# bderembl/msom

Measured on NVIDIA B200. Metric: cell-layer updates/s, higher is better.
Workload: dtype f64

## Files before the change

### include/msqg.h

```cpp
#ifndef MSQG_H
#define MSQG_H

#ifdef __cplusplus
extern "C" {
#endif

#define MSQG_MAXL 32

enum {
  MSQG_OK = 0,
  MSQG_ERR_ARG = -1,
  MSQG_ERR_CUDA = -2,
  MSQG_ERR_FILE = -3,
  MSQG_ERR_CONFIG = -4,
  MSQG_ERR_NOCONV = -5
};

typedef struct msqg_params {
  int N, nl, ediag, varRo, nptr, flsrv;
  double L0, Rom, Ekb, Eks, tau0, Re, Re4, sbc, beta, afilt, Lfmax;
  double DT, tend, dtout, dtflt, CFL;
  double Fr[MSQG_MAXL], dh[MSQG_MAXL], upg[MSQG_MAXL], vpg[MSQG_MAXL];
  double iRe, iRe4;
  int stochastic;
// ... 86 lines not shown
int msqg_filter_de_pm(msqg_model *m, double dtflt, double ediag, int pm_field);
int msqg_energy_tend(msqg_model *m, double dt, double ediag);
int msqg_reset_energy(msqg_model *m);
int msqg_tendency_bfn(msqg_model *m, double direction);
int msqg_bfn_direction(msqg_model *m, double direction);
double msqg_get_ts_previous(msqg_model *m);
void msqg_set_ts_previous(msqg_model *m, double v);
void msqg_seed_noise(msqg_model *m, unsigned seed);
int msqg_set_noise_mode(msqg_model *m, int mode);
long msqg_launch_count(msqg_model *m);
const char *msqg_last_error(void);

int msqg_set_keep_dq(msqg_model *m, int keep);
int msqg_set_dissipation(msqg_model *m, double iRe, double iRe4, double Eks, double Ekb);
void msqg_derive_params(msqg_params *p);

int msqg_test_relax(msqg_model *m, int level, double *a, const double *b, int nsweeps);
int msqg_test_relax_scalar(msqg_model *m, int level, double lambda, double *a, const double *b, int nsweeps);
int msqg_test_residual(msqg_model *m, const double *a, const double *b, double *res, double *maxres);
int msqg_test_residual_levels(msqg_model *m, int mode, const double *a, const double *b, double *out, double *maxres,
                              int *bottom);
int msqg_test_restrict(msqg_model *m, int level, const double *fine, double *coarse);
int msqg_test_prolong(msqg_model *m, int level, const double *coarse, double *fine);
int msqg_test_div(int device, const double *x, const double *d, double *q_fast, double *q_ieee, int n);
int msqg_profile_enable(msqg_model *m, int on);
int msqg_profile_read(msqg_model *m, double *ms, long *count, long *aux_sum);
int msqg_test_relax_profile(msqg_model *m, int level, int nsweeps, long long *out, int max_workers);
int msqg_time_vcycle(msqg_model *m, int nrelax, int reps, double *ms_out);

typedef struct msqg_ensemble msqg_ensemble;
int msqg_ensemble_create(const msqg_params *p, int device, int nmembers, const unsigned *seeds ,
                         int noise_mode, int smoother, msqg_ensemble **out);
void msqg_ensemble_destroy(msqg_ensemble *e);
int msqg_ensemble_size(msqg_ensemble *e);
msqg_model *msqg_ensemble_member(msqg_ensemble *e, int k);
int msqg_ensemble_set_const(msqg_ensemble *e);
int msqg_ensemble_step(msqg_ensemble *e, int nsteps, double *dt_last );
double msqg_ensemble_time(msqg_ensemble *e, int k);

typedef struct msqg_group msqg_group;
int msqg_nccl_unique_id(void *out128);
int msqg_group_create_local(const msqg_params *p, int device, int px, int py, int agg_n, msqg_group **out);
int msqg_group_create_nccl(const msqg_params *p, int device, int px, int py, int agg_n, int rank, int nranks,
                           const void *uid128, msqg_group **out);
int msqg_group_create_local_sm(const msqg_params *p, int device, int px, int py, int agg_n, int smoother, msqg_group **out);
int msqg_group_create_nccl_sm(const msqg_params *p, int device, int px, int py, int agg_n, int smoother, int rank, int nranks,
// ... 67 lines not shown
```

### msom_b200/capi.py

```python
import ctypes as C
import os

import numpy as np

_HERE = os.path.dirname(os.path.abspath(__file__))
LIB_CUDA = os.path.join(_HERE, "lib", "libmsqg_cuda.so")
MAXL = 32

(PSI, Q, PSIPG, FR, QFORC, TOPO, RD, SSTOCH, ZETA, DQ, STR, NSTOCH, IBU, CL2M, CM2L, PM, QM, TMP, ZETAP,
 QPRED, SIGFILT, DE_BF, DE_VD, DE_J1, DE_J2, DE_J3, DE_FT, PO_MFT, PTR, PTR_RELAX, DPTR, QOF, SIGLEV) = range(33)

OK, ERR_ARG, ERR_CUDA, ERR_FILE, ERR_CONFIG, ERR_NOCONV = 0, -1, -2, -3, -4, -5


class Params(C.Structure):
    _fields_ = (
        [(k, C.c_int) for k in ("N", "nl", "ediag", "varRo", "nptr", "flsrv")]
        + [(k, C.c_double) for k in ("L0", "Rom", "Ekb", "Eks", "tau0", "Re", "Re4", "sbc", "beta",
                                     "afilt", "Lfmax", "DT", "tend", "dtout", "dtflt", "CFL")]
        + [(k, C.c_double * MAXL) for k in ("Fr", "dh", "upg", "vpg")]
        + [("iRe", C.c_double), ("iRe4", C.c_double), ("stochastic", C.c_int),
           ("tr_stoch", C.c_double), ("itr_stoch", C.c_double), ("amp_stoch", C.c_double),
           ("mode_pv_invert", C.c_int)]
        + [(k, C.c_double * MAXL) for k in ("ptr_r", "Pe", "ptr_ir", "iPe")]
# ... 80 lines not shown
    L.msqg_invertq.argtypes = [vp, C.c_int]
    L.msqg_comp_q.argtypes = [vp]
    L.msqg_last_mgstats.argtypes = [vp, C.c_int, C.POINTER(MgStats)]
    L.msqg_total_cycles.argtypes = [vp]
    L.msqg_total_cycles.restype = C.c_long
    L.msqg_update.argtypes = [vp, C.c_int, C.c_double, pd]
    L.msqg_advance.argtypes = [vp, C.c_int, C.c_int, C.c_double]
    L.msqg_step.argtypes = [vp, C.c_double, C.c_double, pd, pd]
    L.msqg_ke1.argtypes = [vp, pd]
    L.msqg_tendency_bfn.argtypes = [vp, C.c_double]
    L.msqg_get_ts_previous.argtypes = [vp]
    L.msqg_get_ts_previous.restype = C.c_double
    L.msqg_set_ts_previous.argtypes = [vp, C.c_double]
    L.msqg_seed_noise.argtypes = [vp, C.c_uint]
    L.msqg_set_noise_mode.argtypes = [vp, C.c_int]
    L.msqg_launch_count.argtypes = [vp]
    L.msqg_launch_count.restype = C.c_long
    L.msqg_test_relax.argtypes = [vp, C.c_int, dp, dp, C.c_int]
    L.msqg_test_relax_scalar.argtypes = [vp, C.c_int, C.c_double, dp, dp, C.c_int]
    L.msqg_test_residual.argtypes = [vp, dp, dp, dp, pd]
    L.msqg_test_residual_levels.argtypes = [vp, C.c_int, dp, dp, dp, pd, C.POINTER(C.c_int)]
    L.msqg_test_restrict.argtypes = [vp, C.c_int, dp, dp]
    L.msqg_test_prolong.argtypes = [vp, C.c_int, dp, dp]
    L.msqg_test_div.argtypes = [C.c_int, dp, dp, dp, dp, C.c_int]
    L.msqg_time_vcycle.argtypes = [vp, C.c_int, C.c_int, pd]
    L.msqg_profile_enable.argtypes = [vp, C.c_int]
    L.msqg_profile_read.argtypes = [vp, pd, C.POINTER(C.c_long), C.POINTER(C.c_long)]
    L.msqg_reset_field.argtypes = [vp, C.c_int]
    _lib = L
    return L


def check(rc):
    if rc != 0:
        raise MsqgError(rc, lib().msqg_last_error().decode(errors="replace"))


def make_params(**kw):
    p = Params()
    lib().msqg_default_params(C.byref(p))
    for k, v in kw.items():
        if k in ("Fr", "dh", "upg", "vpg", "ptr_r", "Pe"):
            arr = getattr(p, k)
            for i, x in enumerate(v):
                arr[i] = float(x)
        else:
# ... 32 lines not shown
            if self.owned:
                self.L.msqg_destroy(self.h)
            self.h = None

    def __del__(self):
        try:
            self.close()
        except Exception:
            pass

    def nfields(self, fid):
        return self.L.msqg_nfields(self.h, fid)

    def set(self, fid, arr):
        arr = np.ascontiguousarray(arr, dtype=np.float64)
        assert arr.shape == (self.nfields(fid), self.N, self.N), (arr.shape, self.nfields(fid))
        check(self.L.msqg_set_field(self.h, fid, arr))

    def get(self, fid):
        out = np.zeros((self.nfields(fid), self.N, self.N))
        check(self.L.msqg_get_field(self.h, fid, out))
        return out

    def set_async(self, fid, pinned):
        check(self.L.msqg_set_field_async(self.h, fid, pinned))

    def commit(self):
        check(self.L.msqg_set_field_commit(self.h))

    def get_async(self, fid, pinned):
        check(self.L.msqg_get_field_async(self.h, fid, pinned))

    def io_wait(self):
        check(self.L.msqg_io_wait(self.h))

    def set_smoother(self, name):
        check(self.L.msqg_set_smoother(self.h, {"lex": 0, "rb": 1}[name]))

    def set_energy_conserv(self, on):
        check(self.L.msqg_set_energy_conserv(self.h, int(bool(on))))

    def set_const(self):
        check(self.L.msqg_set_const(self.h))

    def invertq(self, q_id=Q):
        check(self.L.msqg_invertq(self.h, q_id))
# ... 67 lines not shown
```

### msom_b200/csrc/model.cu

```cuda
#include "../../include/msqg.h"
#include "layout.cuh"
#include "mg_kernels.cuh"
#include "rb_kernels.cuh"
#include "rhs_kernels.cuh"

#include <cmath>
#include <cstdio>
#include <cstdlib>
#include <cstring>
#include <dlfcn.h>
#include <vector>
#include <utility>
#include <map>
#include <tuple>
#include <thread>
#include <mutex>
#include <condition_variable>
#include <string>
#include <atomic>

static thread_local char g_err[512] = "";
static std::mutex g_kernel_init_mu;
extern "C" const char *msqg_last_error(void) { return g_err; }
#define FAIL(code, ...)                        \
// ... 1147 lines not shown
static inline cudaError_t zero_words(cudaStream_t st, double *p, int n) {
  k_zero_words<<<1, 64, 0, st>>>(p, n);
  return cudaGetLastError();
}

static int check_relax_err(msqg_model *m) {
  CK(to_host(m->stream, m->h_err, m->d_err, 1));
  CK(cudaStreamSynchronize(m->stream));
  if (*m->h_err) {
    CK(cudaMemsetAsync(m->d_err, 0, sizeof(int), m->stream));
    k_fill_u64<<<m->num_sms * 4, 256, 0, m->stream>>>(m->mailbox, m->mailbox_words, MAIL_EMPTY);
    FAIL(MSQG_ERR_CUDA, "relax wavefront timed out waiting on a neighbour strip");
  }
  return MSQG_OK;
}

struct MgProblem {
  int nf;
  int mode;
  double *a;
  const double *b;
};

static int residual_pyr_bottom(const msqg_model *m) {
  const int D = m->depth;
  if (m->g[D].bc != 0 || m->periodic || D < 2) return D;
  return D - PYR_MAXLEV > 1 ? D - PYR_MAXLEV : 1;
}

static int mg_residual_enqueue(msqg_model *m, const MgProblem &P) {
  const int D = m->depth;
  const Geom &g = m->g[D];
  CK(zero_words(m->stream, m->d_scal, 1));
  const int bottom = residual_pyr_bottom(m);
  if (bottom < D) {
    PyrLevels L;
    L.nlev = D - bottom;
    for (int k = 0; k < PYR_MAXLEV; k++) {
      const int l = k < L.nlev ? D - 1 - k : D;
      L.p[k] = m->res.lev[l]; L.pitch[k] = m->g[l].pitch; L.plane[k] = m->g[l].plane; L.n[k] = m->g[l].nx;
    }
    const dim3 b(32, 8), grid((g.nx + PYR_TILE - 1) / PYR_TILE, (g.ny + PYR_TILE - 1) / PYR_TILE);
    const LayerMetrics M = metrics_of(m);
    StretchConsts S;
    for (int l = 0; l < MSQG_NLMAX; l++) S.s[l] = l < m->nl ? m->s_lev[(size_t)D * m->nl + l] : 0.;
    { ProfScope ps(m, PROF_RESIDUAL, 0);
    if (P.mode >= 0) {
      k_residual_pyr<1, true><<<grid, b, 0, m->stream>>>(P.a, P.b, m->res.lev[D], m->ibu.lev[D] + (size_t)P.mode * g.plane, S, g, M, L, m->d_scal);
    } else if (m->s_uniform) {
      NL_SWITCH(m->nl, k_residual_pyr<NL, false><<<grid, b, 0, m->stream>>>(P.a, P.b, m->res.lev[D], nullptr, S, g, M, L, m->d_scal));
    } else {
      NL_SWITCH(m->nl, k_residual_pyr<NL, true><<<grid, b, 0, m->stream>>>(P.a, P.b, m->res.lev[D], m->str.lev[D], S, g, M, L, m->d_scal));
    }
    }
    m->launches++;
    CK(cudaGetLastError());
    CK(to_host(m->stream, m->h_scal, m->d_scal, 1));
    return MSQG_OK;
  }
  dim3 b(64, 4);
  { ProfScope ps(m, PROF_RESIDUAL, 0);
  if (P.mode < 0) {
    LayerMetrics M = metrics_of(m);
    NL_SWITCH(m->nl, k_residual<NL><<<grid2(g.nx, g.ny, b), b, 0, m->stream>>>(P.a, P.b, m->res.lev[D], m->str.lev[D], g, M, m->d_scal));
  } else {
    k_residual_scalar<<<grid2(g.nx, g.ny, b), b, 0, m->stream>>>(P.a, P.b, m->res.lev[D], m->ibu.lev[D] + (size_t)P.mode * g.plane, g, m->d_scal);
  }
  }
// ... 196 lines not shown
      ModeMat<NL> M;
      for (int k = 0; k < NL * NL; k++) M.a[k] = m->h_cm2l[k];
      k_project<NL><<<grid2(g.nx, g.ny, b), b, 0, m->stream>>>(m->pm.lev[D], m->psi.lev[D], g, M, matf_m2l, 1);
    });
    m->launches++;
    CK(cudaGetLastError());
  }
  return MSQG_OK;
}
extern "C" int msqg_invertq(msqg_model *m, int q_id) {
  CK(cudaSetDevice(m->device));
  List *L = list_by_id(m, q_id);
  if (!L || L->nf != m->nl) FAIL(MSQG_ERR_ARG, "bad q list");
  if (m->group) return pg_invertq(m->group, m, q_id);
  return invertq_list(m, *L);
}

extern "C" int msqg_comp_q(msqg_model *m) {
  CK(cudaSetDevice(m->device));
  if (m->group) { int rc = pg_halo(m->group, MSQG_PSI); if (rc) return rc; }
  const Geom &g = m->g[m->depth];
  dim3 b(64, 4);
  LayerMetrics M = metrics_of(m);
  NL_SWITCH(m->nl, k_comp_q<NL><<<grid2(g.nx, g.ny, b), b, 0, m->stream>>>(m->psi.lev[m->depth], m->str.lev[m->depth], m->q.lev[m->depth], g, M));
  m->launches++;
  CK(cudaGetLastError());
  return MSQG_OK;
}

typedef void (*dgeev_fn)(const char *, const char *, const int *, double *, const int *, double *, double *, double *,
                         const int *, double *, const int *, double *, const int *, int *, size_t, size_t);
static dgeev_fn find_dgeev() {
  static dgeev_fn fn = nullptr;
  static bool tried = false;
  if (tried) return fn;
  tried = true;
  const char *cands[] = {getenv("MSQG_LAPACK"), "liblapack.so.3", "liblapack.so", "libopenblas.so.0", "libopenblas.so"};
  for (const char *c : cands) {
    if (!c) continue;
    void *h = dlopen(c, RTLD_NOW | RTLD_GLOBAL);
    if (!h) continue;
    fn = (dgeev_fn)dlsym(h, "dgeev_");
    if (!fn) fn = (dgeev_fn)dlsym(h, "scipy_dgeev_");
    if (fn) break;
  }
  return fn;
}
// ... 269 lines not shown
  return MSQG_OK;
}

extern "C" int msqg_set_const(msqg_model *m) {
  if (m->group) return pg_set_const(m->group);
  int rc = set_const_local(m);
  if (rc) return rc;
  return set_const_finish(m);
}

static double timestep_chain(msqg_model *m, double umax, double dtmax, double Delta) {
  const double CFL = m->p.CFL;
  dtmax /= CFL;
  if (umax != 0.) {
    const double dt = Delta / umax;
    if (dt < dtmax) dtmax = dt;
  }
  dtmax *= CFL;
  if (dtmax > m->ts_previous) dtmax = (m->ts_previous + 0.1 * dtmax) / 1.1;
  m->ts_previous = dtmax;
  return dtmax;
}

static int rhs_prepare(msqg_model *m) {
  const int D = m->depth;
  const Geom &g = m->g[D];
  dim3 b(64, 4);
  CK(zero_words(m->stream, m->d_scal + 1, m->nl));
  ProfScope ps(m, PROF_LAP, 0);
  launch_lap(m->stream, m->nl, m->psi.lev[D], m->zeta.lev[D], g, m->d_scal + 1, m->sbcc);
  m->launches++;
  if (m->iRe != 0. || m->iRe4 != 0.) {
    launch_lap(m->stream, m->nl, m->zeta.lev[D], m->tmp.lev[D], g, nullptr, m->sbcc);
    m->launches++;
  }
  CK(cudaGetLastError());
  CK(to_host(m->stream, m->h_scal + 1, m->d_scal + 1, m->nl));
  return MSQG_OK;
}
static double dt_chain(msqg_model *m, double dtmax) {
  const double Delta = m->g[m->depth].Delta;
  for (int l = 0; l < m->nl; l++) {
    dtmax = timestep_chain(m, m->h_scal[1 + l], dtmax, Delta);
    dtmax = timestep_chain(m, m->umax_pg[l], dtmax, Delta);
  }
  return dtmax;
}

static int rhs_launch(msqg_model *m, List &q_ev, const double *q_in, double *q_out, double *dq, double dt, float dts) {
  const int D = m->depth;
  const Geom &g = m->g[D];
  const int nl = m->nl;
  RhsArgs A;
  memset(&A, 0, sizeof(A));
  A.psi = m->psi.lev[D]; A.zeta = m->zeta.lev[D]; A.tmp = m->tmp.lev[D]; A.pp = m->psipg.lev[D];
  A.zp = m->zetap.lev[D]; A.s = m->str.lev[D]; A.qforc = m->has_qforc ? m->qforc.lev[D] : nullptr;
  A.topo = m->topo.lev[D]; A.ro = m->ro.lev[D];
  A.q_in = q_in; A.q_ev = q_ev.lev[D]; A.q_out = q_out; A.dq = dq;
  A.noise = m->p.stochastic ? m->nstoch.lev[D] : nullptr;
  A.wind = m->d_wind; A.g = g;
  for (int l = 0; l < nl; l++) { A.idh0[l] = m->idh0[l]; A.idh1[l] = m->idh1[l]; }
  A.beta = m->p.beta; A.iRe = m->iRe; A.iRe4 = m->iRe4;
  A.ceks = m->Eks / (m->p.Rom * 2 * m->dhf[0]);
  A.cekb = m->Ekb / (m->p.Rom * 2 * m->dhf[nl - 1]);
  A.dhb = m->dhf[nl - 1];
  A.dt = dt; A.itr = m->p.itr_stoch; A.dts = dts;
  A.has_pg = m->has_pg; A.has_zp = m->has_zp; A.use_tmp = (m->iRe != 0. || m->iRe4 != 0.);
  A.flag_topo = m->flag_topo; A.stochastic = m->p.stochastic;
  A.econs = (m->econs && !m->p.stochastic) ? 1 : 0;
  if (A.econs) {
    if (g.bc) FAIL(MSQG_ERR_ARG, "the ENERGY_CONSERV variant is not available on decomposed grids");
    dim3 bg(32, 8);
    k_ghosts<<<grid2(g.nx + 2, g.ny + 2, bg, nl), bg, 0, m->stream>>>(q_ev.lev[D], nl, g, -1.);
    m->launches++;
  }
  ProfScope ps(m, PROF_RHS, 0);
  static int rhs_variant = -1;
  if (rhs_variant < 0) { const char *e = getenv("MSQG_RHS"); rhs_variant = (e && !strcmp(e, "gather")) ? 0 : 1; }
  if (rhs_variant == 1 && !A.has_pg && !A.has_zp && !A.flag_topo && !A.stochastic && !A.econs) {
    dim3 bt(RT_X, RT_Y);
    NL_SWITCH(nl, k_rhs_t<NL><<<grid2(g.nx, g.ny, bt), bt, 0, m->stream>>>(A));
  } else {
    dim3 b(32, 4);
    NL_SWITCH(nl, k_rhs<NL><<<grid2(g.nx, g.ny, b), b, 0, m->stream>>>(A));
  }
  m->launches++;
  CK(cudaGetLastError());
  return MSQG_OK;
}

static int ptr_launch(msqg_model *m, List &tr, const double *tr_in, double *tr_out, double *dptr, double dt) {
  if (m->p.nptr <= 0) return MSQG_OK;
  if (m->g[m->depth].bc) FAIL(MSQG_ERR_ARG, "passive tracers are not supported on decomposed grids");
  const int D = m->depth;
  const Geom &g = m->g[D];
  PtrArgs A;
  memset(&A, 0, sizeof(A));
  A.psi = m->psi.lev[D]; A.ptr = tr.lev[D]; A.relax = m->ptr_relax.lev[D];
  A.ptr_in = tr_in; A.ptr_out = tr_out; A.dptr = dptr; A.g = g; A.dt = dt; A.nptr = m->p.nptr;
  for (int nt = 0; nt < m->p.nptr; nt++) { A.iPe[nt] = m->p.iPe[nt]; A.ptr_ir[nt] = m->p.ptr_ir[nt]; }
  dim3 b(64, 4);
  k_ptr_rhs<<<grid2(g.nx, g.ny, b, tr.nf), b, 0, m->stream>>>(A);
  m->launches++;
  CK(cudaGetLastError());
// ... 293 lines not shown
  launch_lap(m->stream, nl, m->psi.lev[D], m->zeta.lev[D], g, nullptr, m->sbcc);
  m->launches++;
  if (m->iRe != 0. || m->iRe4 != 0.) {
    launch_lap(m->stream, nl, m->zeta.lev[D], m->tmp.lev[D], g, nullptr, m->sbcc);
    m->launches++;
  }
  EnergyArgs A;
  memset(&A, 0, sizeof(A));
  A.psi = m->psi.lev[D]; A.zeta = m->zeta.lev[D]; A.tmp = m->tmp.lev[D]; A.pp = m->psipg.lev[D];
  A.zp = m->zetap.lev[D]; A.s = m->str.lev[D];
  A.de_bf = m->de_bf.lev[D]; A.de_vd = m->de_vd.lev[D]; A.de_j1 = m->de_j1.lev[D]; A.de_j2 = m->de_j2.lev[D];
  A.de_j3 = m->de_j3.lev[D]; A.po_mft = m->po_mft.lev[D];
  A.g = g;
  for (int l = 0; l < nl; l++) { A.idh0[l] = m->idh0[l]; A.idh1[l] = m->idh1[l]; }
  A.beta = m->p.beta; A.iRe = m->iRe; A.iRe4 = m->iRe4;
  A.ceks = m->Eks / (m->p.Rom * 2 * m->dhf[0]);
  A.cekb = m->Ekb / (m->p.Rom * 2 * m->dhf[nl - 1]);
  A.dt = dt; A.ediag = ediag;
  A.has_pg = m->has_pg; A.has_zp = m->has_zp; A.nme_ft = m->nme_ft;
  if (m->econs) {
    if (!m->tmp2.nf && (rc = alloc_list(m, m->tmp2, nl, -1., D, D))) return rc;
    dim3 bq(64, 4);
    LayerMetrics M = metrics_of(m);
    NL_SWITCH(nl, k_comp_q<NL><<<grid2(g.nx, g.ny, bq), bq, 0, m->stream>>>(m->psi.lev[D], m->str.lev[D], m->tmp2.lev[D], g, M));
    m->launches++;
    A.qt = m->tmp2.lev[D];
  }
  dim3 b(32, 4);
  NL_SWITCH(nl, k_energy<NL><<<grid2(g.nx, g.ny, b), b, 0, m->stream>>>(A));
  m->launches++;
  CK(cudaGetLastError());
  m->nme_ft += 1;
  return MSQG_OK;
}

extern "C" int msqg_ke1(msqg_model *m, double *ke) {
  CK(cudaSetDevice(m->device));
  const Geom &g = m->g[m->depth];
  dim3 b(16, 16);
  dim3 gr = grid2(g.nx, g.ny, b);
  k_ke_partial<<<gr, b, 0, m->stream>>>(m->psi.lev[m->depth], g, m->d_kepart);
  m->launches++;
  CK(cudaGetLastError());
  std::vector<double> part((size_t)gr.x * gr.y);
  CK(cudaMemcpyAsync(part.data(), m->d_kepart, part.size() * sizeof(double), cudaMemcpyDeviceToHost, m->stream));
  CK(cudaStreamSynchronize(m->stream));
  double s = 0.;
// ... 16 lines not shown
  CK(cudaStreamSynchronize(m->stream));
  (void)dt_chain(m, m->p.DT);
  return MSQG_OK;
}

static int upload_level(msqg_model *m, double *dst, const double *host, int nf, int lev, double sg) {
  const Geom &g = m->g[lev];
  size_t cnt = (size_t)nf * g.nx * g.ny;
  if (cnt > m->stage_doubles) FAIL(MSQG_ERR_ARG, "staging buffer too small");
  CK(cudaMemcpyAsync(m->d_stage, host, cnt * sizeof(double), cudaMemcpyHostToDevice, m->stream));
  dim3 b(32, 8);
  k_pack<<<grid2(g.nx + 2, g.ny + 2, b, nf), b, 0, m->stream>>>(dst, m->d_stage, nf, g, sg);
  CK(cudaGetLastError());
  CK(cudaStreamSynchronize(m->stream));
  return MSQG_OK;
}
static int download_level(msqg_model *m, double *host, const double *src, int nf, int lev) {
  const Geom &g = m->g[lev];
  size_t cnt = (size_t)nf * g.nx * g.ny;
  dim3 b(32, 8);
  k_unpack<<<grid2(g.nx, g.ny, b, nf), b, 0, m->stream>>>(m->d_stage, src, nf, g);
  CK(cudaGetLastError());
  CK(cudaMemcpyAsync(host, m->d_stage, cnt * sizeof(double), cudaMemcpyDeviceToHost, m->stream));
  CK(cudaStreamSynchronize(m->stream));
  return MSQG_OK;
}

extern "C" int msqg_test_relax(msqg_model *m, int level, double *a, const double *b, int nsweeps) {
  CK(cudaSetDevice(m->device));
  if (level < 1 || level > m->depth) FAIL(MSQG_ERR_ARG, "bad level");
  if (!m->const_set || !m->s_uniform) FAIL(MSQG_ERR_ARG, "needs set_const and uniform stretching");
  int rc;
  if ((rc = upload_level(m, m->da.lev[level], a, m->nl, level, -1.))) return rc;
  if ((rc = upload_level(m, m->res.lev[level], b, m->nl, level, -1.))) return rc;
  NL_SWITCH(m->nl, { auto C = relax_coef_layers<NL>(m, level); rc = launch_relax<NL>(m, m->da.lev[level], m->res.lev[level], level, nsweeps, C); });
  if (rc) return rc;
  if ((rc = check_relax_err(m))) return rc;
  return download_level(m, a, m->da.lev[level], m->nl, level);
}
extern "C" int msqg_test_relax_scalar(msqg_model *m, int level, double lambda, double *a, const double *b, int nsweeps) {
  CK(cudaSetDevice(m->device));
  if (level < 1 || level > m->depth) FAIL(MSQG_ERR_ARG, "bad level");
  int rc;
  if ((rc = upload_level(m, m->da.lev[level], a, 1, level, -1.))) return rc;
  if ((rc = upload_level(m, m->res.lev[level], b, 1, level, -1.))) return rc;
  auto C = relax_coef_scalar(m, level, lambda);
// ... 240 lines not shown
```

### msom_b200/csrc/rhs_kernels.cuh

```cuda
#pragma once
#include "layout.cuh"
#include "mg_kernels.cuh"

__device__ __forceinline__ double lapf(double fac, const double *__restrict__ p, size_t c, int pitch, const Geom &g) {
  return div_by(fac * (p[c + 1] + p[c - 1] + p[c + pitch] + p[c - pitch] - 4 * p[c]), g.D2, g.rD2);
}
__device__ __forceinline__ double lap5(const double *__restrict__ p, size_t c, int pitch, const Geom &g) {
  return div_by(p[c + 1] + p[c - 1] + p[c + pitch] + p[c - pitch] - 4 * p[c], g.D2, g.rD2);
}

__device__ __forceinline__ void write_ghosts(double *__restrict__ p, const Geom &g, int x, int y, double v, double sg) {
  const int nx = g.nx, ny = g.ny;
  const bool l = x == 0, r = x == nx - 1, bo = y == 0, t = y == ny - 1;
  if (l) p[GIDX(g.pitch, y, -1)] = sg * v;
  if (r) p[GIDX(g.pitch, y, nx)] = sg * v;
  if (bo) p[GIDX(g.pitch, -1, x)] = sg * v;
  if (t) p[GIDX(g.pitch, ny, x)] = sg * v;
  if (l && bo) p[GIDX(g.pitch, -1, -1)] = v;
  if (l && t) p[GIDX(g.pitch, ny, -1)] = v;
  if (r && bo) p[GIDX(g.pitch, -1, nx)] = v;
  if (r && t) p[GIDX(g.pitch, ny, nx)] = v;
}

__global__ void __launch_bounds__(256)
// ... 114 lines not shown
#define PO(a, b) po[cc + (a) + (b) * P]
#define QO(a, b) qo[cc + (a) + (b) * P]
  return div_by(((QO(1, 0) - QO(-1, 0)) * (PO(0, 1) - PO(0, -1))
         + (QO(0, -1) - QO(0, 1)) * (PO(1, 0) - PO(-1, 0))
         + QO(1, 0) * (PO(1, 1) - PO(1, -1))
         - QO(-1, 0) * (PO(-1, 1) - PO(-1, -1))
         - QO(0, 1) * (PO(1, 1) - PO(-1, 1))
         + QO(0, -1) * (PO(1, -1) - PO(-1, -1))
         + PO(0, 1) * (QO(1, 1) - QO(-1, 1))
         - PO(0, -1) * (QO(1, -1) - QO(-1, -1))
         - PO(1, 0) * (QO(1, 1) - QO(1, -1))
         + PO(-1, 0) * (QO(-1, 1) - QO(-1, -1))),
        G.D12, G.rD12);
#undef PO
#undef QO
}

struct RhsArgs {
  const double *psi, *zeta, *tmp, *pp, *zp, *s, *qforc, *topo, *ro, *sstoch_unused;
  const double *q_in;
  const double *q_ev;
  double *q_out;
  double *dq;
  const double *noise;
  const double *wind;
  Geom g;
  double idh0[MSQG_NLMAX], idh1[MSQG_NLMAX];
  double beta, iRe, iRe4, ceks, cekb;
  double dhb;
  double dt, itr;
  float dts;
  int has_pg, has_zp, use_tmp, flag_topo, stochastic;
  int econs;
};

#ifndef RHS_MINB
#define RHS_MINB 6
#endif
template <int NL>
__global__ void __launch_bounds__(128, RHS_MINB)
k_rhs(RhsArgs A) {
  const int x = blockIdx.x * blockDim.x + threadIdx.x;
  const int y = blockIdx.y * blockDim.y + threadIdx.y;
  const Geom g = A.g;
  if (x >= g.nx || y >= g.ny) return;
  const size_t c = GIDX(g.pitch, y, x);
  const int P = g.pitch;
  const size_t pl = g.plane;
  double jd = 0., ju;
#pragma unroll
// ... 50 lines not shown
      }
      dq = 1. * dq + lapf(A.iRe4, t1, c, P, g);
    }
    if (l == 0) dq -= A.ceks * qo[c];
    if (l == NL - 1) dq -= A.cekb * qo[c];
    if (l == 0) dq -= A.wind[y];
    if (A.qforc) dq += A.qforc[l * pl + c];
    if (l == NL - 1 && A.flag_topo) dq += jac(po, A.topo, c, P, g) / (A.ro[c] * A.dhb);
    if (A.dq) A.dq[l * pl + c] = dq;
    if (A.q_out) {
      double v;
      if (!A.stochastic)
        v = A.q_in[l * pl + c] + dq * A.dt;
      else
        v = A.q_in[l * pl + c] + dq * A.dt + A.noise[l * pl + c] * A.dts;
      A.q_out[l * pl + c] = v;
    }
  }
}

#define RT_X 32
#define RT_Y 8
#define RT_P (RT_X + 2)
struct TileAcc {
  const double *t;
  __device__ __forceinline__ double operator()(int a, int b) const { return t[a + b * RT_P]; }
};
template <class PA, class QA>
__device__ __forceinline__ double jac_acc(const PA PO, const QA QO, const Geom &G) {
  return div_by(((QO(1, 0) - QO(-1, 0)) * (PO(0, 1) - PO(0, -1))
         + (QO(0, -1) - QO(0, 1)) * (PO(1, 0) - PO(-1, 0))
         + QO(1, 0) * (PO(1, 1) - PO(1, -1))
         - QO(-1, 0) * (PO(-1, 1) - PO(-1, -1))
         - QO(0, 1) * (PO(1, 1) - PO(-1, 1))
         + QO(0, -1) * (PO(1, -1) - PO(-1, -1))
         + PO(0, 1) * (QO(1, 1) - QO(-1, 1))
         - PO(0, -1) * (QO(1, -1) - QO(-1, -1))
         - PO(1, 0) * (QO(1, 1) - QO(1, -1))
         + PO(-1, 0) * (QO(-1, 1) - QO(-1, -1))),
        G.D12, G.rD12);
}
__device__ __forceinline__ void rt_load(double *__restrict__ tile, const double *__restrict__ src, const Geom &g, int x0, int y0, int tid) {
  constexpr int NE = (RT_Y + 2) * RT_P, NT = RT_X * RT_Y;
#pragma unroll
  for (int k = 0; k < (NE + NT - 1) / NT; k++) {
    const int e = tid + k * NT;
    const int ry = e / RT_P, rx = e - ry * RT_P;
    const int gx = x0 - 1 + rx, gy = y0 - 1 + ry;
    if (e < NE && gx <= g.nx && gy <= g.ny)
      asm volatile("cp.async.ca.shared.global [%0], [%1], 8;\n" ::"r"((unsigned)__cvta_generic_to_shared(tile + e)), "l"(src + GIDX(g.pitch, gy, gx)) : "memory");
  }
}
template <int NL>
__global__ void __launch_bounds__(RT_X * RT_Y)
k_rhs_t(RhsArgs A) {
  constexpr int TS = (RT_Y + 2) * RT_P;
  __shared__ double sp[3][TS], sz[3][TS], st[3][TS];
  const Geom g = A.g;
  const int x0 = blockIdx.x * RT_X, y0 = blockIdx.y * RT_Y;
  const int tid = threadIdx.y * RT_X + threadIdx.x;
  const int x = x0 + threadIdx.x, y = y0 + threadIdx.y;
  const bool active = x < g.nx && y < g.ny;
  const size_t c = GIDX(g.pitch, active ? y : 0, active ? x : 0);
  const size_t pl = g.plane;
  const int tc = (threadIdx.y + 1) * RT_P + threadIdx.x + 1;
  auto stage = [&](int l) {
    if (l < NL) {
      rt_load(sp[l % 3], A.psi + l * pl, g, x0, y0, tid);
      rt_load(sz[l % 3], A.zeta + l * pl, g, x0, y0, tid);
      if (A.use_tmp) rt_load(st[l % 3], A.tmp + l * pl, g, x0, y0, tid);
    }
    cp_async_commit();
  };
  stage(0);
  stage(1);
  double jd = 0., ju;
  double zm = 0., tm = 0., sm = 0.;
  double sl = (NL > 1) ? A.s[c] : 0., qi = (A.q_out && active) ? A.q_in[c] : 0.;
#pragma unroll
  for (int l = 0; l < NL; l++) {
    cp_async_wait<0>();
    __syncthreads();
    stage(l + 2);
    if (active) {
      const TileAcc po{sp[l % 3] + tc}, po2{sp[(l + 1) % 3] + tc}, qo{sz[l % 3] + tc};
      const double *t1s = st[l % 3] + tc;
      const double sn = (l + 1 < NL - 1) ? A.s[(l + 1) * pl + c] : 0.;
      const double qn = (A.q_out && l + 1 < NL) ? A.q_in[(l + 1) * pl + c] : 0.;
      double dq = 0.;
      ju = -jd;
      if (l < NL - 1) jd = jac_acc(po, po2, g);
      double adv;
      const double be = div_by(A.beta * (po(-1, 0) - po(1, 0)), g.D2x, g.rD2x);
      adv = jac_acc(po, qo, g);
      adv = adv + be;
      if (l == 0)
        adv = adv + sl * jd * A.idh1[0];
      else if (l < NL - 1)
        adv = adv + sm * ju * A.idh0[l] + sl * jd * A.idh1[l];
      else
        adv = adv + sm * ju * A.idh0[l];
      dq += adv;
      const double zc = qo(0, 0);
      if (A.use_tmp) {
        const double tcv = t1s[0];
        const double zp = (l < NL - 1) ? sz[(l + 1) % 3][tc] : 0., tp = (l < NL - 1) ? st[(l + 1) % 3][tc] : 0.;
        if (l == 0) {
          dq = 1. * dq + A.iRe * sl * (zp - zc) * A.idh1[0];
        } else if (l < NL - 1) {
          dq = 1. * dq + A.iRe * (sm * (zm - zc) * A.idh0[l] + sl * (zp - zc) * A.idh1[l]);
        } else {
          dq = 1. * dq + A.iRe * sm * (zm - zc) * A.idh0[l];
        }
        dq += tcv * A.iRe;
        if (l == 0) {
          dq = 1. * dq + A.iRe4 * sl * (tp - tcv) * A.idh1[0];
        } else if (l < NL - 1) {
          dq = 1. * dq + A.iRe4 * (sm * (tm - tcv) * A.idh0[l] + sl * (tp - tcv) * A.idh1[l]);
        } else {
          dq = 1. * dq + A.iRe4 * sm * (tm - tcv) * A.idh0[l];
        }
        dq = 1. * dq + div_by(A.iRe4 * (t1s[1] + t1s[-1] + t1s[RT_P] + t1s[-RT_P] - 4 * tcv), g.D2, g.rD2);
        tm = tcv;
      }
      zm = zc; sm = sl;
      if (l == 0) dq -= A.ceks * zc;
      if (l == NL - 1) dq -= A.cekb * zc;
      if (l == 0) dq -= A.wind[y];
      if (A.qforc) dq += A.qforc[l * pl + c];
      if (A.dq) A.dq[l * pl + c] = dq;
      if (A.q_out) A.q_out[l * pl + c] = qi + dq * A.dt;
      sl = sn; qi = qn;
    }
  }
  cp_async_wait<0>();
}

struct EnergyArgs {
  const double *psi, *zeta, *tmp, *pp, *zp, *s;
  double *de_bf, *de_vd, *de_j1, *de_j2, *de_j3, *po_mft;
  const double *qt;
  Geom g;
  double idh0[MSQG_NLMAX], idh1[MSQG_NLMAX];
  double beta, iRe, iRe4, ceks, cekb, dt, ediag;
  int has_pg, has_zp, nme_ft;
};

template <int NL>
__global__ void __launch_bounds__(128)
k_energy(EnergyArgs A) {
  const int x = blockIdx.x * blockDim.x + threadIdx.x;
  const int y = blockIdx.y * blockDim.y + threadIdx.y;
  const Geom g = A.g;
  if (x >= g.nx || y >= g.ny) return;
  const size_t c = GIDX(g.pitch, y, x);
  const int P = g.pitch;
// ... 86 lines not shown
  double dp = 0.;
  dp += jac(po, tr, c, g.pitch, g) + lapf(A.iPe[nt], tr, c, g.pitch, g) + A.ptr_ir[nt] * (A.relax[f * pl + c] - tr[c]);
  if (A.dptr) A.dptr[f * pl + c] = dp;
  if (A.ptr_out) {
    const double v = A.ptr_in[f * pl + c] + dp * A.dt;
    A.ptr_out[f * pl + c] = v;
    write_ghosts(A.ptr_out + f * pl, g, x, y, v, 1.);
  }
}

__global__ void k_advance(double *__restrict__ out, const double *__restrict__ in, const double *__restrict__ dq,
                          const double *__restrict__ noise, Geom g, double dt, float dts) {
  const int x = blockIdx.x * blockDim.x + threadIdx.x;
  const int y = blockIdx.y * blockDim.y + threadIdx.y;
  const int f = blockIdx.z;
  if (x >= g.nx || y >= g.ny) return;
  const size_t c = (size_t)f * g.plane + GIDX(g.pitch, y, x);
  if (noise)
    out[c] = in[c] + dq[c] * dt + noise[c] * dts;
  else
    out[c] = in[c] + dq[c] * dt;
}

template <int NL>
__global__ void __launch_bounds__(256)
k_comp_q(const double *__restrict__ psi, const double *__restrict__ s, double *__restrict__ q, Geom g, LayerMetrics M) {
  const int x = blockIdx.x * blockDim.x + threadIdx.x;
  const int y = blockIdx.y * blockDim.y + threadIdx.y;
  if (x >= g.nx || y >= g.ny) return;
  const size_t c = GIDX(g.pitch, y, x);
  const size_t pl = g.plane;
#pragma unroll
  for (int l = 0; l < NL; l++) {
    const double *p = psi + l * pl;
    double v = 0. * 0. + 1. * lap5(p, c, g.pitch, g);
    if (l == 0)
      v = 1. * v + 1. * s[c] * (p[pl + c] - p[c]) * M.idh1[0];
    else if (l < NL - 1)
      v = 1. * v + 1. * (s[(l - 1) * pl + c] * (p[c - pl] - p[c]) * M.idh0[l] + s[l * pl + c] * (p[c + pl] - p[c]) * M.idh1[l]);
    else
      v = 1. * v + 1. * s[(l - 1) * pl + c] * (p[c - pl] - p[c]) * M.idh0[l];
    q[l * pl + c] = v;
    write_ghosts(q + l * pl, g, x, y, v, -1.);
  }
}

template <int NL>
struct ModeMat {
  double a[NL * NL];
};

template <int NL, bool RING = false>
__global__ void __launch_bounds__(256)
k_project(const double *__restrict__ in, double *__restrict__ out, Geom g, ModeMat<NL> M,
          const double *__restrict__ matf , int ghosts) {
  const int x = blockIdx.x * blockDim.x + threadIdx.x - (RING ? 1 : 0);
  const int y = blockIdx.y * blockDim.y + threadIdx.y - (RING ? 1 : 0);
  if (RING) {
    if (x > g.nx || y > g.ny) return;
    const bool okx = x < 0 ? (g.bc & 1) : (x >= g.nx ? (g.bc & 2) : true);
    const bool oky = y < 0 ? (g.bc & 4) : (y >= g.ny ? (g.bc & 8) : true);
    if (!okx || !oky) return;
    ghosts = 0;
  } else if (x >= g.nx || y >= g.ny)
// ... 67 lines not shown
```

Before: 4.197 billion.

## Fuse biharmonic Laplacian into tiled RHS kernel and use uniform stretching constants

The tiled RHS kernel now loads zeta with a two-cell halo and computes the Laplacian of zeta (tmp) in shared memory, so the separate launch_lap pass over zeta is skipped. The kernel still writes tmp and its ghosts out for later users. When stretching is uniform, the s field is passed as per-layer constants instead of being read from global memory in k_rhs_t and k_comp_q. The cost is a larger shared zeta tile, extra halo-recompute threads, and more template variants.

```diff
diff --git a/include/msqg.h b/include/msqg.h
--- a/include/msqg.h
+++ b/include/msqg.h
@@ -132,6 +132,7 @@
                               int *bottom);
 int msqg_test_restrict(msqg_model *m, int level, const double *fine, double *coarse);
 int msqg_test_prolong(msqg_model *m, int level, const double *coarse, double *fine);
+int msqg_test_get_field_ring(msqg_model *m, int id, double *host);
 int msqg_test_div(int device, const double *x, const double *d, double *q_fast, double *q_ieee, int n);
 int msqg_profile_enable(msqg_model *m, int on);
 int msqg_profile_read(msqg_model *m, double *ms, long *count, long *aux_sum);
diff --git a/msom_b200/capi.py b/msom_b200/capi.py
--- a/msom_b200/capi.py
+++ b/msom_b200/capi.py
@@ -126,6 +126,7 @@
     L.msqg_test_residual_levels.argtypes = [vp, C.c_int, dp, dp, dp, pd, C.POINTER(C.c_int)]
     L.msqg_test_restrict.argtypes = [vp, C.c_int, dp, dp]
     L.msqg_test_prolong.argtypes = [vp, C.c_int, dp, dp]
+    L.msqg_test_get_field_ring.argtypes = [vp, C.c_int, dp]
     L.msqg_test_div.argtypes = [C.c_int, dp, dp, dp, dp, C.c_int]
     L.msqg_time_vcycle.argtypes = [vp, C.c_int, C.c_int, pd]
     L.msqg_profile_enable.argtypes = [vp, C.c_int]
@@ -204,6 +205,11 @@
         check(self.L.msqg_get_field(self.h, fid, out))
         return out
 
+    def get_ring(self, fid):
+        out = np.zeros((self.nfields(fid), self.N + 2, self.N + 2))
+        check(self.L.msqg_test_get_field_ring(self.h, fid, out))
+        return out
+
     def set_async(self, fid, pinned):
         check(self.L.msqg_set_field_async(self.h, fid, pinned))
 
diff --git a/msom_b200/csrc/model.cu b/msom_b200/csrc/model.cu
--- a/msom_b200/csrc/model.cu
+++ b/msom_b200/csrc/model.cu
@@ -1193,6 +1193,11 @@
   const double *b;
 };
 
+static StretchConsts stretch_consts(const msqg_model *m, int lev) {
+  StretchConsts S;
+  for (int l = 0; l < MSQG_NLMAX; l++) S.s[l] = l < m->nl ? m->s_lev[(size_t)lev * m->nl + l] : 0.;
+  return S;
+}
 static int residual_pyr_bottom(const msqg_model *m) {
   const int D = m->depth;
   if (m->g[D].bc != 0 || m->periodic || D < 2) return D;
@@ -1213,8 +1218,7 @@
     }
     const dim3 b(32, 8), grid((g.nx + PYR_TILE - 1) / PYR_TILE, (g.ny + PYR_TILE - 1) / PYR_TILE);
     const LayerMetrics M = metrics_of(m);
-    StretchConsts S;
-    for (int l = 0; l < MSQG_NLMAX; l++) S.s[l] = l < m->nl ? m->s_lev[(size_t)D * m->nl + l] : 0.;
+    const StretchConsts S = stretch_consts(m, D);
     { ProfScope ps(m, PROF_RESIDUAL, 0);
     if (P.mode >= 0) {
       k_residual_pyr<1, true><<<grid, b, 0, m->stream>>>(P.a, P.b, m->res.lev[D], m->ibu.lev[D] + (size_t)P.mode * g.plane, S, g, M, L, m->d_scal);
@@ -1457,7 +1461,11 @@
   const Geom &g = m->g[m->depth];
   dim3 b(64, 4);
   LayerMetrics M = metrics_of(m);
-  NL_SWITCH(m->nl, k_comp_q<NL><<<grid2(g.nx, g.ny, b), b, 0, m->stream>>>(m->psi.lev[m->depth], m->str.lev[m->depth], m->q.lev[m->depth], g, M));
+  const int D = m->depth;
+  if (m->s_uniform)
+    NL_SWITCH(m->nl, k_comp_q<NL, true><<<grid2(g.nx, g.ny, b), b, 0, m->stream>>>(m->psi.lev[D], nullptr, m->q.lev[D], g, M, stretch_consts(m, D)))
+  else
+    NL_SWITCH(m->nl, k_comp_q<NL, false><<<grid2(g.nx, g.ny, b), b, 0, m->stream>>>(m->psi.lev[D], m->str.lev[D], m->q.lev[D], g, M, StretchConsts{}))
   m->launches++;
   CK(cudaGetLastError());
   return MSQG_OK;
@@ -1773,15 +1781,23 @@
   return dtmax;
 }
 
+static bool rhs_tiled(const msqg_model *m) {
+  static int rhs_variant = -1;
+  if (rhs_variant < 0) { const char *e = getenv("MSQG_RHS"); rhs_variant = (e && !strcmp(e, "gather")) ? 0 : 1; }
+  return rhs_variant == 1 && !m->has_pg && !m->has_zp && !m->flag_topo && !m->p.stochastic && !m->econs;
+}
+static bool rhs_forms_tmp(const msqg_model *m) {
+  return rhs_tiled(m) && m->g[m->depth].bc == 0 && m->sbcc == 0. && (m->iRe != 0. || m->iRe4 != 0.);
+}
+
 static int rhs_prepare(msqg_model *m) {
   const int D = m->depth;
   const Geom &g = m->g[D];
-  dim3 b(64, 4);
   CK(zero_words(m->stream, m->d_scal + 1, m->nl));
   ProfScope ps(m, PROF_LAP, 0);
   launch_lap(m->stream, m->nl, m->psi.lev[D], m->zeta.lev[D], g, m->d_scal + 1, m->sbcc);
   m->launches++;
-  if (m->iRe != 0. || m->iRe4 != 0.) {
+  if ((m->iRe != 0. || m->iRe4 != 0.) && !rhs_forms_tmp(m)) {
     launch_lap(m->stream, m->nl, m->zeta.lev[D], m->tmp.lev[D], g, nullptr, m->sbcc);
     m->launches++;
   }
@@ -1826,11 +1842,19 @@
     m->launches++;
   }
   ProfScope ps(m, PROF_RHS, 0);
-  static int rhs_variant = -1;
-  if (rhs_variant < 0) { const char *e = getenv("MSQG_RHS"); rhs_variant = (e && !strcmp(e, "gather")) ? 0 : 1; }
-  if (rhs_variant == 1 && !A.has_pg && !A.has_zp && !A.flag_topo && !A.stochastic && !A.econs) {
+  if (rhs_tiled(m)) {
     dim3 bt(RT_X, RT_Y);
-    NL_SWITCH(nl, k_rhs_t<NL><<<grid2(g.nx, g.ny, bt), bt, 0, m->stream>>>(A));
+    const dim3 gr = grid2(g.nx, g.ny, bt);
+    const bool ftmp = rhs_forms_tmp(m);
+    A.tmp_out = ftmp ? m->tmp.lev[D] : nullptr;
+    if (m->s_uniform) {
+      for (int l = 0; l < nl; l++) A.sc[l] = m->s_lev[(size_t)D * nl + l];
+      if (ftmp) NL_SWITCH(nl, k_rhs_t<NL, true, true><<<gr, bt, 0, m->stream>>>(A))
+      else NL_SWITCH(nl, k_rhs_t<NL, false, true><<<gr, bt, 0, m->stream>>>(A))
+    } else {
+      if (ftmp) NL_SWITCH(nl, k_rhs_t<NL, true, false><<<gr, bt, 0, m->stream>>>(A))
+      else NL_SWITCH(nl, k_rhs_t<NL, false, false><<<gr, bt, 0, m->stream>>>(A))
+    }
   } else {
     dim3 b(32, 4);
     NL_SWITCH(nl, k_rhs<NL><<<grid2(g.nx, g.ny, b), b, 0, m->stream>>>(A));
@@ -2170,7 +2194,10 @@
     if (!m->tmp2.nf && (rc = alloc_list(m, m->tmp2, nl, -1., D, D))) return rc;
     dim3 bq(64, 4);
     LayerMetrics M = metrics_of(m);
-    NL_SWITCH(nl, k_comp_q<NL><<<grid2(g.nx, g.ny, bq), bq, 0, m->stream>>>(m->psi.lev[D], m->str.lev[D], m->tmp2.lev[D], g, M));
+    if (m->s_uniform)
+      NL_SWITCH(nl, k_comp_q<NL, true><<<grid2(g.nx, g.ny, bq), bq, 0, m->stream>>>(m->psi.lev[D], nullptr, m->tmp2.lev[D], g, M, stretch_consts(m, D)))
+    else
+      NL_SWITCH(nl, k_comp_q<NL, false><<<grid2(g.nx, g.ny, bq), bq, 0, m->stream>>>(m->psi.lev[D], m->str.lev[D], m->tmp2.lev[D], g, M, StretchConsts{}))
     m->launches++;
     A.qt = m->tmp2.lev[D];
   }
@@ -2233,6 +2260,20 @@
   k_unpack<<<grid2(g.nx, g.ny, b, nf), b, 0, m->stream>>>(m->d_stage, src, nf, g);
   CK(cudaGetLastError());
   CK(cudaMemcpyAsync(host, m->d_stage, cnt * sizeof(double), cudaMemcpyDeviceToHost, m->stream));
+  CK(cudaStreamSynchronize(m->stream));
+  return MSQG_OK;
+}
+
+extern "C" int msqg_test_get_field_ring(msqg_model *m, int id, double *host) {
+  CK(cudaSetDevice(m->device));
+  List *L = list_by_id(m, id);
+  const int D = m->depth;
+  if (!L || !L->nf || !L->lev[D]) FAIL(MSQG_ERR_ARG, "bad or unallocated list");
+  const Geom &g = m->g[D];
+  if (g.bc) FAIL(MSQG_ERR_ARG, "msqg_test_get_field_ring reads an undecomposed model");
+  const size_t w = (size_t)g.nx + 2;
+  CK(cudaMemcpy2DAsync(host, w * sizeof(double), L->lev[D] + GIDX(g.pitch, -1, -1), g.pitch * sizeof(double),
+                       w * sizeof(double), (size_t)L->nf * (g.ny + 2), cudaMemcpyDeviceToHost, m->stream));
   CK(cudaStreamSynchronize(m->stream));
   return MSQG_OK;
 }
diff --git a/msom_b200/csrc/rhs_kernels.cuh b/msom_b200/csrc/rhs_kernels.cuh
--- a/msom_b200/csrc/rhs_kernels.cuh
+++ b/msom_b200/csrc/rhs_kernels.cuh
@@ -160,10 +160,12 @@
   const double *q_ev;
   double *q_out;
   double *dq;
+  double *tmp_out;
   const double *noise;
   const double *wind;
   Geom g;
   double idh0[MSQG_NLMAX], idh1[MSQG_NLMAX];
+  double sc[MSQG_NLMAX];
   double beta, iRe, iRe4, ceks, cekb;
   double dhb;
   double dt, itr;
@@ -260,9 +262,10 @@
 #define RT_X 32
 #define RT_Y 8
 #define RT_P (RT_X + 2)
+template <int TP>
 struct TileAcc {
   const double *t;
-  __device__ __forceinline__ double operator()(int a, int b) const { return t[a + b * RT_P]; }
+  __device__ __forceinline__ double operator()(int a, int b) const { return t[a + b * TP]; }
 };
 template <class PA, class QA>
 __device__ __forceinline__ double jac_acc(const PA PO, const QA QO, const Geom &G) {
@@ -278,22 +281,36 @@
          + PO(-1, 0) * (QO(-1, 1) - QO(-1, -1))),
         G.D12, G.rD12);
 }
+template <int H>
 __device__ __forceinline__ void rt_load(double *__restrict__ tile, const double *__restrict__ src, const Geom &g, int x0, int y0, int tid) {
-  constexpr int NE = (RT_Y + 2) * RT_P, NT = RT_X * RT_Y;
+  constexpr int TP = RT_X + 2 * H, NE = (RT_Y + 2 * H) * TP, NT = RT_X * RT_Y;
 #pragma unroll
   for (int k = 0; k < (NE + NT - 1) / NT; k++) {
     const int e = tid + k * NT;
-    const int ry = e / RT_P, rx = e - ry * RT_P;
-    const int gx = x0 - 1 + rx, gy = y0 - 1 + ry;
-    if (e < NE && gx <= g.nx && gy <= g.ny)
+    const int ry = e / TP, rx = e - ry * TP;
+    const int gx = x0 - H + rx, gy = y0 - H + ry;
+    if (e < NE && gx <= g.nx && gy <= g.ny && (H == 1 || (gx >= -1 && gy >= -1)))
       asm volatile("cp.async.ca.shared.global [%0], [%1], 8;\n" ::"r"((unsigned)__cvta_generic_to_shared(tile + e)), "l"(src + GIDX(g.pitch, gy, gx)) : "memory");
   }
 }
-template <int NL>
+__device__ __forceinline__ double rt_form_tmp(double *__restrict__ t, const double *__restrict__ z, const Geom &g, int x0, int y0, int rx, int ry) {
+  const int gx = x0 - 1 + rx, gy = y0 - 1 + ry;
+  if (gx > g.nx || gy > g.ny) return 0.;
+  const int cx = min(max(gx, 0), g.nx - 1), cy = min(max(gy, 0), g.ny - 1);
+  constexpr int ZP = RT_P + 2;
+  const double *p = z + (cy - y0 + 2) * ZP + (cx - x0 + 2);
+  double v = div_by(p[1] + p[-1] + p[ZP] + p[-ZP] - 4 * p[0], g.D2, g.rD2);
+  if ((gx != cx) != (gy != cy)) v = -1. * v;
+  t[ry * RT_P + rx] = v;
+  return v;
+}
+template <int NL, bool FTMP, bool SU>
 __global__ void __launch_bounds__(RT_X * RT_Y)
 k_rhs_t(RhsArgs A) {
   constexpr int TS = (RT_Y + 2) * RT_P;
-  __shared__ double sp[3][TS], sz[3][TS], st[3][TS];
+  constexpr int ZH = FTMP ? 2 : 1, ZP = RT_X + 2 * ZH, ZS = (RT_Y + 2 * ZH) * ZP;
+  constexpr int NTB = FTMP ? 2 : 3;
+  __shared__ double sp[3][TS], sz[3][ZS], st[NTB][TS];
   const Geom g = A.g;
   const int x0 = blockIdx.x * RT_X, y0 = blockIdx.y * RT_Y;
   const int tid = threadIdx.y * RT_X + threadIdx.x;
@@ -301,29 +318,54 @@
   const bool active = x < g.nx && y < g.ny;
   const size_t c = GIDX(g.pitch, active ? y : 0, active ? x : 0);
   const size_t pl = g.plane;
-  const int tc = (threadIdx.y + 1) * RT_P + threadIdx.x + 1;
+  const int tc = (threadIdx.y + 1) * RT_P + threadIdx.x + 1, tz = (threadIdx.y + ZH) * ZP + threadIdx.x + ZH;
+  const bool use_tmp = FTMP || A.use_tmp;
   auto stage = [&](int l) {
     if (l < NL) {
-      rt_load(sp[l % 3], A.psi + l * pl, g, x0, y0, tid);
-      rt_load(sz[l % 3], A.zeta + l * pl, g, x0, y0, tid);
-      if (A.use_tmp) rt_load(st[l % 3], A.tmp + l * pl, g, x0, y0, tid);
+      rt_load<1>(sp[l % 3], A.psi + l * pl, g, x0, y0, tid);
+      rt_load<ZH>(sz[l % 3], A.zeta + l * pl, g, x0, y0, tid);
+      if (!FTMP && A.use_tmp) rt_load<1>(st[l % 3], A.tmp + l * pl, g, x0, y0, tid);
     }
     cp_async_commit();
+  };
+  auto sfield = [&](int l) -> double { return SU ? A.sc[l] : A.s[l * pl + c]; };
+  auto form_tmp = [&](int l) -> double {
+    double *t = st[l % NTB];
+    const double v = rt_form_tmp(t, sz[l % 3], g, x0, y0, threadIdx.x + 1, threadIdx.y + 1);
+    if (active) {
+      double *o = A.tmp_out + l * pl;
+      o[c] = v;
+      write_ghosts(o, g, x, y, v, -1.);
+    }
+    static_assert(RT_X == 32 && RT_Y <= 16, "one warp per block row; the side columns fit half a warp");
+    if (threadIdx.y < 2)
+      rt_form_tmp(t, sz[l % 3], g, x0, y0, threadIdx.x + 1, threadIdx.y == 0 ? 0 : RT_Y + 1);
+    else if (threadIdx.y == 2 && threadIdx.x < 2 * RT_Y)
+      rt_form_tmp(t, sz[l % 3], g, x0, y0, threadIdx.x < RT_Y ? 0 : RT_X + 1, 1 + threadIdx.x % RT_Y);
+    return v;
   };
   stage(0);
   stage(1);
   double jd = 0., ju;
   double zm = 0., tm = 0., sm = 0.;
-  double sl = (NL > 1) ? A.s[c] : 0., qi = (A.q_out && active) ? A.q_in[c] : 0.;
+  double sl = (NL > 1) ? sfield(0) : 0., qi = (A.q_out && active) ? A.q_in[c] : 0.;
+  double tl = 0.;
+  if (FTMP) {
+    cp_async_wait<1>();
+    __syncthreads();
+    tl = form_tmp(0);
+  }
 #pragma unroll
   for (int l = 0; l < NL; l++) {
     cp_async_wait<0>();
     __syncthreads();
     stage(l + 2);
+    const double tn = (FTMP && l < NL - 1) ? form_tmp(l + 1) : 0.;
     if (active) {
-      const TileAcc po{sp[l % 3] + tc}, po2{sp[(l + 1) % 3] + tc}, qo{sz[l % 3] + tc};
-      const double *t1s = st[l % 3] + tc;
-      const double sn = (l + 1 < NL - 1) ? A.s[(l + 1) * pl + c] : 0.;
+      const TileAcc<RT_P> po{sp[l % 3] + tc}, po2{sp[(l + 1) % 3] + tc};
+      const TileAcc<ZP> qo{sz[l % 3] + tz};
+      const double *t1s = st[l % NTB] + tc;
+      const double sn = (l + 1 < NL - 1) ? sfield(l + 1) : 0.;
       const double qn = (A.q_out && l + 1 < NL) ? A.q_in[(l + 1) * pl + c] : 0.;
       double dq = 0.;
       ju = -jd;
@@ -340,9 +382,10 @@
         adv = adv + sm * ju * A.idh0[l];
       dq += adv;
       const double zc = qo(0, 0);
-      if (A.use_tmp) {
-        const double tcv = t1s[0];
-        const double zp = (l < NL - 1) ? sz[(l + 1) % 3][tc] : 0., tp = (l < NL - 1) ? st[(l + 1) % 3][tc] : 0.;
+      if (use_tmp) {
+        const double tcv = FTMP ? tl : t1s[0];
+        const double zp = (l < NL - 1) ? sz[(l + 1) % 3][tz] : 0.;
+        const double tp = FTMP ? tn : ((l < NL - 1) ? st[(l + 1) % NTB][tc] : 0.);
         if (l == 0) {
           dq = 1. * dq + A.iRe * sl * (zp - zc) * A.idh1[0];
         } else if (l < NL - 1) {
@@ -370,6 +413,7 @@
       if (A.q_out) A.q_out[l * pl + c] = qi + dq * A.dt;
       sl = sn; qi = qn;
     }
+    tl = tn;
   }
   cp_async_wait<0>();
 }
@@ -502,24 +546,25 @@
     out[c] = in[c] + dq[c] * dt;
 }
 
-template <int NL>
+template <int NL, bool SU>
 __global__ void __launch_bounds__(256)
-k_comp_q(const double *__restrict__ psi, const double *__restrict__ s, double *__restrict__ q, Geom g, LayerMetrics M) {
+k_comp_q(const double *__restrict__ psi, const double *__restrict__ s, double *__restrict__ q, Geom g, LayerMetrics M, StretchConsts S) {
   const int x = blockIdx.x * blockDim.x + threadIdx.x;
   const int y = blockIdx.y * blockDim.y + threadIdx.y;
   if (x >= g.nx || y >= g.ny) return;
   const size_t c = GIDX(g.pitch, y, x);
   const size_t pl = g.plane;
+  auto sf = [&](int l) -> double { return SU ? S.s[l] : s[l * pl + c]; };
 #pragma unroll
   for (int l = 0; l < NL; l++) {
     const double *p = psi + l * pl;
     double v = 0. * 0. + 1. * lap5(p, c, g.pitch, g);
     if (l == 0)
-      v = 1. * v + 1. * s[c] * (p[pl + c] - p[c]) * M.idh1[0];
+      v = 1. * v + 1. * sf(0) * (p[pl + c] - p[c]) * M.idh1[0];
     else if (l < NL - 1)
-      v = 1. * v + 1. * (s[(l - 1) * pl + c] * (p[c - pl] - p[c]) * M.idh0[l] + s[l * pl + c] * (p[c + pl] - p[c]) * M.idh1[l]);
+      v = 1. * v + 1. * (sf(l - 1) * (p[c - pl] - p[c]) * M.idh0[l] + sf(l) * (p[c + pl] - p[c]) * M.idh1[l]);
     else
-      v = 1. * v + 1. * s[(l - 1) * pl + c] * (p[c - pl] - p[c]) * M.idh0[l];
+      v = 1. * v + 1. * sf(l - 1) * (p[c - pl] - p[c]) * M.idh0[l];
     q[l * pl + c] = v;
     write_ghosts(q + l * pl, g, x, y, v, -1.);
   }
```

Result: faster. 4.286 billion, median of 6 (+2.1%).
